# facebookresearch/jepa

Measured on NVIDIA H100. Metric: clips/sec ViT-L/16 16x224^2 synthetic V-JEPA pre-training step, higher is better.
Workload: dtype bf16

## Files before the change

### __graft_entry__.py

```python
import os
import sys

ROOT = os.path.dirname(os.path.abspath(__file__))
if ROOT not in sys.path:
    sys.path.insert(0, ROOT)


def build():
    from jepa_b200 import build as b
    b.build()
    import subprocess
    subprocess.check_call(["make", "-s", "-C", os.path.join(ROOT, "tests", "native"), "all", "test_xattn"])
    import jepa_b200
    from jepa_b200 import _lib
    _lib.load()
    import oracle.vjepa_oracle


def smoke():
    import torch
    sys.path.insert(0, os.path.join(ROOT, "tests"))
    sys.path.insert(0, os.path.join(ROOT, "tests", "golden"))
    from parity_util import run_c1_step_cuda, run_c1_step_oracle, compare_step
    assert torch.cuda.is_available(), "smoke() needs cuda:0"
    dev = torch.device("cuda:0")
    got = run_c1_step_cuda(dev, batch=1, depth_limit=2)
    ref = run_c1_step_oracle(batch=1, depth_limit=2)
    compare_step(got, ref, verbose=True)
    print("smoke OK: loss", got["loss_jepa"], "oracle", ref["loss_jepa"])


if __name__ == "__main__":
    build()
    if len(sys.argv) > 1 and sys.argv[1] == "smoke":
        smoke()
```

### jepa_b200/csrc/gemm.cu

```cuda

#include <stdlib.h>

#include "common.cuh"
#include "vjepa_b200.h"
#include "wgmma.cuh"

namespace vj {

constexpr int BM = 128;
constexpr int BK = 64;
constexpr int kGemmThreads = 384;
constexpr int kPromoteKB = 4;

struct GemmParams {
  int M, N, K;
  int tiles_m, tiles_n, split_k, kb_total, kb_per_split;
  int stream_k;
  long long sk_chunk;
  const float* bias;
  int epi;
  const void* aux;
  long long ldaux;
  const int* aux_rowmap;
  int aux_period;
  void* aux_out;
  long long ldauxout;
  void* D;
  long long ldd;
  int reduce_add;
  float alpha;
};

template <int BN>
struct GemmCfg {
  static constexpr int A_BYTES = BM * BK * 2;
  static constexpr int B_BYTES = BN * BK * 2;
  static constexpr int STAGE_BYTES = A_BYTES + B_BYTES;
  static constexpr int STAGES = BN == 256 ? 4 : (BN == 128 ? 6 : 8);
  static constexpr int BAR_OFF = STAGES * STAGE_BYTES;
  static constexpr int SMEM_BYTES = BAR_OFF + 2 * STAGES * 8 + 1024;
  static_assert(SMEM_BYTES <= 232448, "GEMM shared memory budget exceeded");
};

struct WorkCursor {
  long long cur, end;
};
VJ_DEVINL WorkCursor work_begin(const GemmParams& p) {
  WorkCursor c;
  if (p.stream_k) {
    const long long total_kb = (long long)p.tiles_m * p.tiles_n * p.kb_total;
    c.cur = (long long)blockIdx.x * p.sk_chunk;
    c.end = min(total_kb, c.cur + p.sk_chunk);
  } else {
    c.cur = blockIdx.x;
    c.end = (long long)p.tiles_m * p.tiles_n * p.split_k;
  }
  return c;
}
VJ_DEVINL bool work_next(const GemmParams& p, WorkCursor& c, int& t, int& kb0, int& kb1) {
  if (c.cur >= c.end) return false;
  if (p.stream_k) {
    t = int(c.cur / p.kb_total);
    kb0 = int(c.cur - (long long)t * p.kb_total);
    const long long take = min((long long)(p.kb_total - kb0), c.end - c.cur);
    kb1 = kb0 + int(take);
    c.cur += take;
  } else {
    const int tiles = p.tiles_m * p.tiles_n;
    const int split = int(c.cur / tiles);
    t = int(c.cur - (long long)split * tiles);
    kb0 = split * p.kb_per_split;
    kb1 = min(p.kb_total, kb0 + p.kb_per_split);
    c.cur += gridDim.x;
  }
  return true;
}

VJ_DEVINL float erf_as(float x) {
  const float ax = fabsf(x);
  const float t = __fdividef(1.0f, fmaf(0.3275911f, ax, 1.0f));
  float poly = fmaf(1.061405429f, t, -1.453152027f);
  poly = fmaf(poly, t, 1.421413741f);
  poly = fmaf(poly, t, -0.284496736f);
  poly = fmaf(poly, t, 0.254829592f);
  poly *= t;
  const float r = 1.0f - poly * __expf(-ax * ax);
  return copysignf(r, x);
}
VJ_DEVINL float gelu_and_grad(float x, float& d) {
  const float cdf = 0.5f * (1.0f + erf_as(x * 0.70710678118654752f));
  const float pdf = 0.39894228040143268f * __expf(-0.5f * x * x);
  d = fmaf(x, pdf, cdf);
  return x * cdf;
}
VJ_DEVINL float gelu_grad_fast(float x) {
  float d;
  gelu_and_grad(x, d);
  return d;
}

template <int BN, bool A_MN, bool B_MN, bool OUT_F32, int EPI, bool AUX32>
__global__ void __launch_bounds__(kGemmThreads, 1)
gemm_kernel(const __grid_constant__ CUtensorMap tmA, const __grid_constant__ CUtensorMap tmB, const GemmParams p) {
  constexpr bool kUsesAux = (EPI == VJ_EPI_ADD || EPI == VJ_EPI_DGELU || EPI == VJ_EPI_MUL);
  using Cfg = GemmCfg<BN>;
  constexpr int STAGES = Cfg::STAGES;
  extern __shared__ uint8_t smem_raw[];
  uint8_t* smem = reinterpret_cast<uint8_t*>((reinterpret_cast<uintptr_t>(smem_raw) + 1023) & ~uintptr_t(1023));
  uint64_t* bars = reinterpret_cast<uint64_t*>(smem + Cfg::BAR_OFF);
  const uint32_t full0 = smem_u32(bars);
  const uint32_t empty0 = smem_u32(bars + STAGES);
  const int wg = threadIdx.x >> 7;

  if (threadIdx.x == 0) {
    for (int s = 0; s < STAGES; ++s) {
      mbar_init(full0 + 8 * s, 1);
      mbar_init(empty0 + 8 * s, 8);
    }
    fence_mbar_init();
    tma_prefetch_desc(&tmA);
    tma_prefetch_desc(&tmB);
  }
  __syncthreads();

  if (wg == 0) {
    setmaxnreg_dec<40>();
    if (threadIdx.x == 0) {
      int stage = 0;
      uint32_t phase = 0;
      WorkCursor wc = work_begin(p);
      int t, kb0, kb1;
      while (work_next(p, wc, t, kb0, kb1)) {
        const int m0 = (t / p.tiles_n) * BM;
        const int n0 = (t % p.tiles_n) * BN;
        for (int kb = kb0; kb < kb1; ++kb) {
          mbar_wait(empty0 + 8 * stage, phase ^ 1);
          const uint32_t sa = smem_u32(smem + stage * Cfg::STAGE_BYTES);
          const uint32_t sb = sa + Cfg::A_BYTES;
          const uint32_t fb = full0 + 8 * stage;
          mbar_expect_tx(fb, Cfg::STAGE_BYTES);
          const int k0 = kb * BK;
          if (!A_MN) {
            tma_load_2d(sa, &tmA, fb, k0, m0);
          } else {
#pragma unroll
            for (int j = 0; j < BM / 64; ++j) tma_load_2d(sa + j * 8192, &tmA, fb, m0 + 64 * j, k0);
          }
          if (!B_MN) {
            tma_load_2d(sb, &tmB, fb, k0, n0);
          } else {
#pragma unroll
            for (int j = 0; j < BN / 64; ++j) tma_load_2d(sb + j * 8192, &tmB, fb, n0 + 64 * j, k0);
          }
          if (++stage == STAGES) {
            stage = 0;
            phase ^= 1;
          }
        }
      }
    }
    return;
  }

  setmaxnreg_inc<232>();
  const int cw = wg - 1;
  const int warp_in_wg = (threadIdx.x >> 5) & 3;
  const int lane = threadIdx.x & 31;
  constexpr bool kPromote = A_MN && B_MN;
  static_assert(!kPromote || BN <= 128, "promoted accumulation needs two accumulator sets in registers");
  int stage = 0;
  uint32_t phase = 0;
  float acc[BN / 2];
  float part[kPromote ? BN / 2 : 1];
  WorkCursor wc = work_begin(p);
  int t, kb0, kb1;
  while (work_next(p, wc, t, kb0, kb1)) {
    const int m0 = (t / p.tiles_n) * BM;
    const int n0 = (t % p.tiles_n) * BN;
    if constexpr (kPromote) {
#pragma unroll
      for (int i = 0; i < BN / 2; ++i) acc[i] = 0.f;
    }
    int prev = -1;
    for (int kb = kb0; kb < kb1; ++kb) {
      mbar_wait(full0 + 8 * stage, phase);
      const uint32_t sa = smem_u32(smem + stage * Cfg::STAGE_BYTES) + cw * 8192;
      const uint32_t sb = smem_u32(smem + stage * Cfg::STAGE_BYTES) + Cfg::A_BYTES;
      const uint64_t da0 = A_MN ? make_smem_desc(sa, 8192, 1024, 1) : make_smem_desc(sa, 16, 1024, 1);
      const uint64_t db0 = B_MN ? make_smem_desc(sb, 8192, 1024, 1) : make_smem_desc(sb, 16, 1024, 1);
      if constexpr (kPromote) {
        const bool group_first = (kb - kb0) % kPromoteKB == 0;
        const bool group_last = (kb - kb0) % kPromoteKB == kPromoteKB - 1 || kb + 1 == kb1;
        wgmma_fence_regs(part);
        wgmma_fence();
#pragma unroll
        for (int kk = 0; kk < BK / 16; ++kk)
          wgmma_ss<BN, 1, 1>(part, da0 + ((kk * 2048) >> 4), db0 + ((kk * 2048) >> 4), (!group_first || kk > 0) ? 1 : 0);
        wgmma_commit();
        if (group_last) {
          wgmma_wait<0>();
          wgmma_fence_regs(part);
#pragma unroll
          for (int i = 0; i < BN / 2; ++i) acc[i] += part[i];
        } else {
          wgmma_wait<1>();
        }
      } else {
        wgmma_fence_regs(acc);
        wgmma_fence();
#pragma unroll
        for (int kk = 0; kk < BK / 16; ++kk) {
          const uint32_t koa = A_MN ? kk * 2048 : kk * 32, kob = B_MN ? kk * 2048 : kk * 32;
          wgmma_ss<BN, A_MN ? 1 : 0, B_MN ? 1 : 0>(acc, da0 + (koa >> 4), db0 + (kob >> 4), (kb > kb0 || kk > 0) ? 1 : 0);
        }
        wgmma_commit();
        wgmma_wait<1>();
        wgmma_fence_regs(acc);
      }
      if (prev >= 0) {
        __syncwarp();
        if (lane == 0) mbar_arrive(empty0 + 8 * prev);
      }
      prev = stage;
      if (++stage == STAGES) {
        stage = 0;
        phase ^= 1;
      }
    }
    wgmma_wait<0>();
    wgmma_fence_regs(acc);
    __syncwarp();
    if (lane == 0) mbar_arrive(empty0 + 8 * prev);

    const bool add_bias = p.bias != nullptr && kb0 == 0;
    const int r0 = m0 + cw * 64 + warp_in_wg * 16 + (lane >> 2);
    const int cq = n0 + 2 * (lane & 3);
#pragma unroll
    for (int h = 0; h < 2; ++h) {
      const int row = r0 + 8 * h;
      if (row >= p.M) continue;
      long long arow = row;
      if (kUsesAux && AUX32) {
        if (p.aux_rowmap != nullptr) arow = p.aux_rowmap[row];
        else if (p.aux_period > 0) arow = row % p.aux_period;
      }
#pragma unroll
      for (int j = 0; j < BN / 8; ++j) {
        const int col = cq + 8 * j;
        float v0 = acc[4 * j + 2 * h] * p.alpha, v1 = acc[4 * j + 2 * h + 1] * p.alpha;
        if (add_bias) {
          const float2 b = __ldg(reinterpret_cast<const float2*>(p.bias + col));
          v0 += b.x;
          v1 += b.y;
        }
        if (kUsesAux) {
          float x0, x1;
          if (AUX32) {
            const float2 x = __ldg(reinterpret_cast<const float2*>(reinterpret_cast<const float*>(p.aux) + arow * p.ldaux + col));
            x0 = x.x; x1 = x.y;
          } else {
            const uint32_t x = __ldg(reinterpret_cast<const unsigned int*>(reinterpret_cast<const __nv_bfloat16*>(p.aux) +
                                                                             arow * p.ldaux + col));
            x0 = bf16_lo(x); x1 = bf16_hi(x);
          }
          if (EPI == VJ_EPI_ADD) { v0 += x0; v1 += x1; }
          else if (EPI == VJ_EPI_MUL) { v0 *= x0; v1 *= x1; }
          else { v0 *= gelu_grad_fast(x0); v1 *= gelu_grad_fast(x1); }
        }
        if (EPI == VJ_EPI_GELU || EPI == VJ_EPI_GELU_GRAD) {
          float d0, d1;
          const float g0 = gelu_and_grad(v0, d0), g1 = gelu_and_grad(v1, d1);
          if (p.aux_out != nullptr) {
            const uint32_t o = EPI == VJ_EPI_GELU ? pack_bf16x2(v0, v1) : pack_bf16x2(d0, d1);
            *reinterpret_cast<uint32_t*>(reinterpret_cast<__nv_bfloat16*>(p.aux_out) + (long long)row * p.ldauxout + col) = o;
          }
          v0 = g0;
          v1 = g1;
        }
        if (OUT_F32) {
          float2* dst = reinterpret_cast<float2*>(reinterpret_cast<float*>(p.D) + (long long)row * p.ldd + col);
          if (p.reduce_add) atomicAdd(dst, make_float2(v0, v1));
          else *dst = make_float2(v0, v1);
        } else {
          *reinterpret_cast<uint32_t*>(reinterpret_cast<__nv_bfloat16*>(p.D) + (long long)row * p.ldd + col) =
              pack_bf16x2(v0, v1);
        }
      }
    }
  }
}

template <int BN, bool A_MN, bool B_MN, bool OUT_F32, int EPI, bool AUX32 = false>
static int launch_gemm(const CUtensorMap& tA, const CUtensorMap& tB, const GemmParams& p, cudaStream_t stream) {
  using Cfg = GemmCfg<BN>;
  auto kern = gemm_kernel<BN, A_MN, B_MN, OUT_F32, EPI, AUX32>;
  static bool configured = false;
  if (!configured) {
    VJ_CUDA(cudaFuncSetAttribute(kern, cudaFuncAttributeMaxDynamicSharedMemorySize, Cfg::SMEM_BYTES));
    configured = true;
  }
  const int total = p.tiles_m * p.tiles_n * p.split_k;
  int grid = total < sm_budget() ? total : sm_budget();
  if (p.stream_k) {
    const long long total_kb = (long long)p.tiles_m * p.tiles_n * p.kb_total;
    grid = int((total_kb + p.sk_chunk - 1) / p.sk_chunk);
  }
  kern<<<grid, kGemmThreads, Cfg::SMEM_BYTES, stream>>>(tA, tB, p);
  VJ_CUDA(cudaGetLastError());
  vj::count_launch(1);
  return 0;
}

template <int BN>
static int dispatch_major(int a_mn, int b_mn, int out_f32, int epi, int aux_f32, const CUtensorMap& tA,
                          const CUtensorMap& tB, const GemmParams& p, cudaStream_t s) {
  if (!a_mn && !b_mn) {
    if (epi == VJ_EPI_NONE) return out_f32 ? launch_gemm<BN, false, false, true, VJ_EPI_NONE>(tA, tB, p, s)
                                           : launch_gemm<BN, false, false, false, VJ_EPI_NONE>(tA, tB, p, s);
    if (epi == VJ_EPI_ADD) {
      if (aux_f32) return out_f32 ? launch_gemm<BN, false, false, true, VJ_EPI_ADD, true>(tA, tB, p, s)
                                  : launch_gemm<BN, false, false, false, VJ_EPI_ADD, true>(tA, tB, p, s);
      if (!out_f32) return launch_gemm<BN, false, false, false, VJ_EPI_ADD, false>(tA, tB, p, s);
    }
    if (epi == VJ_EPI_GELU && !out_f32) return launch_gemm<BN, false, false, false, VJ_EPI_GELU>(tA, tB, p, s);
    if (epi == VJ_EPI_GELU_GRAD && !out_f32) return launch_gemm<BN, false, false, false, VJ_EPI_GELU_GRAD>(tA, tB, p, s);
    if (epi == VJ_EPI_DGELU && !out_f32 && !aux_f32) return launch_gemm<BN, false, false, false, VJ_EPI_DGELU>(tA, tB, p, s);
  } else if (!a_mn && b_mn) {
    if (epi == VJ_EPI_NONE) return out_f32 ? launch_gemm<BN, false, true, true, VJ_EPI_NONE>(tA, tB, p, s)
                                           : launch_gemm<BN, false, true, false, VJ_EPI_NONE>(tA, tB, p, s);
    if (epi == VJ_EPI_DGELU && !out_f32 && !aux_f32) return launch_gemm<BN, false, true, false, VJ_EPI_DGELU>(tA, tB, p, s);
    if (epi == VJ_EPI_MUL && !out_f32 && !aux_f32) return launch_gemm<BN, false, true, false, VJ_EPI_MUL>(tA, tB, p, s);
  } else if (a_mn && b_mn) {
    if constexpr (BN <= 128) {
      if (epi == VJ_EPI_NONE) return out_f32 ? launch_gemm<BN, true, true, true, VJ_EPI_NONE>(tA, tB, p, s)
                                             : launch_gemm<BN, true, true, false, VJ_EPI_NONE>(tA, tB, p, s);
    }
  }
  set_error("vj_gemm: combination a_mn=%d b_mn=%d d_f32=%d epi=%d is not instantiated", a_mn, b_mn, out_f32, epi);
  return -1;
}

}

extern "C" int vj_gemm(const void* A, long long lda, int a_mn, const void* B, long long ldb,
                       int b_mn, void* D, long long ldd, int d_f32, int M, int N, int K,
                       const float* bias, float alpha, int epi, const void* aux, long long ldaux,
                       int aux_f32, const int* aux_rowmap, int aux_period, void* aux_out,
                       long long ldauxout, int split_k, int accumulate, void* stream_) {
  using namespace vj;
  cudaStream_t stream = reinterpret_cast<cudaStream_t>(stream_);
  VJ_CHECK_ARG(A && B && D, "vj_gemm: null operand");
  VJ_CHECK_ARG(M > 0 && N > 0 && K > 0, "vj_gemm: empty problem M=%d N=%d K=%d", M, N, K);
  VJ_CHECK_ARG(N % 64 == 0, "vj_gemm: N=%d must be a multiple of 64", N);
  VJ_CHECK_ARG(lda % 8 == 0 && ldb % 8 == 0, "vj_gemm: lda/ldb must be multiples of 8 elements (16-byte rows)");
  VJ_CHECK_ARG(ldd % (d_f32 ? 4 : 8) == 0, "vj_gemm: ldd misaligned");
  VJ_CHECK_ARG((reinterpret_cast<uintptr_t>(A) & 15) == 0 && (reinterpret_cast<uintptr_t>(B) & 15) == 0 &&
                   (reinterpret_cast<uintptr_t>(D) & 15) == 0,
               "vj_gemm: operands must be 16-byte aligned");
  VJ_CHECK_ARG(epi >= VJ_EPI_NONE && epi <= VJ_EPI_GELU_GRAD, "vj_gemm: bad epilogue %d", epi);
  VJ_CHECK_ARG(!(accumulate || split_k > 1 || split_k < 0) || d_f32, "vj_gemm: accumulate/split-K needs fp32 D");
  VJ_CHECK_ARG(split_k >= 0 || (epi == VJ_EPI_NONE && accumulate), "vj_gemm: stream-K (split_k < 0) is for accumulating fp32 GEMMs");
  if (epi == VJ_EPI_ADD || epi == VJ_EPI_DGELU || epi == VJ_EPI_MUL) {
    VJ_CHECK_ARG(aux != nullptr, "vj_gemm: epilogue %d needs aux", epi);
    VJ_CHECK_ARG((reinterpret_cast<uintptr_t>(aux) & 15) == 0 && ldaux % (aux_f32 ? 4 : 8) == 0,
                 "vj_gemm: aux misaligned");
  }
  if (a_mn) VJ_CHECK_ARG(M % 8 == 0, "vj_gemm: MN-major A needs M %% 8 == 0");

  const int BN = (N % 256 == 0 && !(a_mn && b_mn)) ? 256 : (N % 128 == 0 ? 128 : 64);
  GemmParams p;
  p.M = M; p.N = N; p.K = K;
  p.tiles_m = (M + BM - 1) / BM;
  p.tiles_n = N / BN;
  p.kb_total = (K + BK - 1) / BK;
  p.stream_k = 0;
  p.sk_chunk = 0;
  if (split_k < 0) {
    const long long total_kb = (long long)p.tiles_m * p.tiles_n * p.kb_total;
    const long long ctas = total_kb < sm_budget() ? total_kb : sm_budget();
    p.stream_k = 1;
    p.sk_chunk = (total_kb + ctas - 1) / ctas;
    split_k = 1;
  }
  if (split_k < 1) split_k = 1;
  if (split_k > p.kb_total) split_k = p.kb_total;
  p.kb_per_split = (p.kb_total + split_k - 1) / split_k;
  p.split_k = (p.kb_total + p.kb_per_split - 1) / p.kb_per_split;
  p.bias = bias;
  p.epi = epi;
  p.aux = aux; p.ldaux = ldaux; p.aux_rowmap = aux_rowmap; p.aux_period = aux_period;
  p.aux_out = (epi == VJ_EPI_GELU || epi == VJ_EPI_GELU_GRAD) ? aux_out : nullptr;
  p.ldauxout = ldauxout;
  p.D = D; p.ldd = ldd;
  p.reduce_add = (accumulate || p.split_k > 1 || p.stream_k) ? 1 : 0;
  p.alpha = alpha;

  if (p.aux_out != nullptr)
    VJ_CHECK_ARG((reinterpret_cast<uintptr_t>(aux_out) & 3) == 0 && ldauxout % 2 == 0, "vj_gemm: aux_out misaligned");
  if ((epi == VJ_EPI_ADD || epi == VJ_EPI_DGELU || epi == VJ_EPI_MUL) && !aux_f32) {
    VJ_CHECK_ARG(aux_rowmap == nullptr && aux_period == 0, "vj_gemm: row-mapped / periodic aux must be fp32");
    VJ_CHECK_ARG(p.split_k == 1, "vj_gemm: aux epilogues do not combine with split-K");
  }
  CUtensorMap tA, tB;
  int rc;
  if (!a_mn) rc = make_tmap_2d(&tA, A, 0, K, M, lda * 2, 64, 128, 3);
  else       rc = make_tmap_2d(&tA, A, 0, M, K, lda * 2, 64, 64, 3);
  if (rc) return rc;
  if (!b_mn) rc = make_tmap_2d(&tB, B, 0, K, N, ldb * 2, 64, BN, 3);
  else       rc = make_tmap_2d(&tB, B, 0, N, K, ldb * 2, 64, 64, 3);
  if (rc) return rc;
  switch (BN) {
    case 256: return dispatch_major<256>(a_mn, b_mn, d_f32, epi, aux_f32, tA, tB, p, stream);
    case 128: return dispatch_major<128>(a_mn, b_mn, d_f32, epi, aux_f32, tA, tB, p, stream);
    default:  return dispatch_major<64>(a_mn, b_mn, d_f32, epi, aux_f32, tA, tB, p, stream);
  }
}
```

Before: 100.7.

## Add ping-pong consumer schedule and TMA-staged epilogue to GEMM kernel

Splits the GEMM kernel into a ping-pong variant, where two consumer warpgroups alternate tiles and hand off through named barriers, and a cooperative BN=256 variant used for long-K problems. The bf16 epilogue now stages results in swizzled shared memory and writes them with TMA stores. A producer thread prefetches bf16 aux tiles via TMA. The goal is to overlap one tile's epilogue with the next tile's MMA mainloop and to coalesce output writes. The cost is more shared memory for staging (fewer pipeline stages for some configs) and more complex synchronization. Weight-gradient (MN-major) GEMMs move to a separate kernel.

```diff
diff --git a/__graft_entry__.py b/__graft_entry__.py
--- a/__graft_entry__.py
+++ b/__graft_entry__.py
@@ -10,7 +10,8 @@
     from jepa_b200 import build as b
     b.build()
     import subprocess
-    subprocess.check_call(["make", "-s", "-C", os.path.join(ROOT, "tests", "native"), "all", "test_xattn"])
+    subprocess.check_call(["make", "-s", "-C", os.path.join(ROOT, "tests", "native"), "all", "test_xattn",
+                           "test_gemm_sched"])
     import jepa_b200
     from jepa_b200 import _lib
     _lib.load()
diff --git a/jepa_b200/csrc/gemm.cu b/jepa_b200/csrc/gemm.cu
--- a/jepa_b200/csrc/gemm.cu
+++ b/jepa_b200/csrc/gemm.cu
@@ -1,5 +1,6 @@
 
 #include <stdlib.h>
+#include <string.h>
 
 #include "common.cuh"
 #include "vjepa_b200.h"
@@ -10,6 +11,7 @@
 constexpr int BM = 128;
 constexpr int BK = 64;
 constexpr int kGemmThreads = 384;
+constexpr int kSmemBudget = 232448;
 constexpr int kPromoteKB = 4;
 
 struct GemmParams {
@@ -36,10 +38,28 @@
   static constexpr int A_BYTES = BM * BK * 2;
   static constexpr int B_BYTES = BN * BK * 2;
   static constexpr int STAGE_BYTES = A_BYTES + B_BYTES;
-  static constexpr int STAGES = BN == 256 ? 4 : (BN == 128 ? 6 : 8);
+  static constexpr int STAGES = BN == 128 ? 6 : 8;
   static constexpr int BAR_OFF = STAGES * STAGE_BYTES;
   static constexpr int SMEM_BYTES = BAR_OFF + 2 * STAGES * 8 + 1024;
-  static_assert(SMEM_BYTES <= 232448, "GEMM shared memory budget exceeded");
+  static_assert(SMEM_BYTES <= kSmemBudget, "GEMM shared memory budget exceeded");
+};
+
+template <int BN, bool STAGED, bool COOP>
+struct PingCfg {
+  static constexpr int ROWS = COOP ? 64 : BM;
+  static constexpr int A_BYTES = BM * BK * 2;
+  static constexpr int B_BYTES = BN * BK * 2;
+  static constexpr int STAGE_BYTES = A_BYTES + B_BYTES;
+  static constexpr int STG_BYTES = STAGED ? ROWS * BN * 2 : 0;
+  static constexpr int BAR_BYTES = 256;
+  static constexpr int FIT = (kSmemBudget - 1024 - BAR_BYTES - 2 * STG_BYTES) / STAGE_BYTES;
+  static constexpr int STAGES = FIT < 8 ? FIT : 8;
+  static constexpr int STG_OFF = STAGES * STAGE_BYTES;
+  static constexpr int BAR_OFF = STG_OFF + 2 * STG_BYTES;
+  static constexpr int SMEM_BYTES = BAR_OFF + BAR_BYTES + 1024;
+  static_assert(STAGES >= 3, "GEMM ring too shallow");
+  static_assert((2 * STAGES + 4) * 8 <= BAR_BYTES, "GEMM barrier block overflow");
+  static_assert(SMEM_BYTES <= kSmemBudget, "GEMM shared memory budget exceeded");
 };
 
 struct WorkCursor {
@@ -98,11 +118,305 @@
   gelu_and_grad(x, d);
   return d;
 }
-
-template <int BN, bool A_MN, bool B_MN, bool OUT_F32, int EPI, bool AUX32>
+template <int EPI>
+VJ_DEVINL void apply_aux(float& v0, float& v1, float x0, float x1) {
+  if (EPI == VJ_EPI_ADD) { v0 += x0; v1 += x1; }
+  else if (EPI == VJ_EPI_MUL) { v0 *= x0; v1 *= x1; }
+  else { v0 *= gelu_grad_fast(x0); v1 *= gelu_grad_fast(x1); }
+}
+VJ_DEVINL int aux32_row(const GemmParams& p, int row) {
+  if (row >= p.M) return 0;
+  if (p.aux_rowmap != nullptr) return p.aux_rowmap[row];
+  if (p.aux_period > 0) return row % p.aux_period;
+  return row;
+}
+
+template <int BN, bool OUT_F32, int EPI, bool AUX32>
+VJ_DEVINL void epilogue_direct(const GemmParams& p, const float (&acc)[BN / 2], int r0, int n0, bool add_bias, int lane) {
+  constexpr bool kUsesAux = (EPI == VJ_EPI_ADD || EPI == VJ_EPI_DGELU || EPI == VJ_EPI_MUL);
+  static_assert(!kUsesAux || AUX32, "bf16 aux goes through the staged epilogue");
+  const int cq = n0 + 2 * (lane & 3);
+#pragma unroll
+  for (int h = 0; h < 2; ++h) {
+    const int row = r0 + (lane >> 2) + 8 * h;
+    if (row >= p.M) continue;
+    const long long arow = kUsesAux ? aux32_row(p, row) : 0;
+#pragma unroll
+    for (int j = 0; j < BN / 8; ++j) {
+      const int col = cq + 8 * j;
+      float v0 = acc[4 * j + 2 * h] * p.alpha, v1 = acc[4 * j + 2 * h + 1] * p.alpha;
+      if (add_bias) {
+        const float2 b = __ldg(reinterpret_cast<const float2*>(p.bias + col));
+        v0 += b.x;
+        v1 += b.y;
+      }
+      if (kUsesAux) {
+        const float2 x = __ldg(reinterpret_cast<const float2*>(reinterpret_cast<const float*>(p.aux) + arow * p.ldaux + col));
+        apply_aux<EPI>(v0, v1, x.x, x.y);
+      }
+      if (OUT_F32) {
+        float2* dst = reinterpret_cast<float2*>(reinterpret_cast<float*>(p.D) + (long long)row * p.ldd + col);
+        if (p.reduce_add) atomicAdd(dst, make_float2(v0, v1));
+        else *dst = make_float2(v0, v1);
+      } else {
+        *reinterpret_cast<uint32_t*>(reinterpret_cast<__nv_bfloat16*>(p.D) + (long long)row * p.ldd + col) =
+            pack_bf16x2(v0, v1);
+      }
+    }
+  }
+}
+
+template <int BN, bool COOP, bool B_MN, bool OUT_F32, int EPI, bool AUX32>
 __global__ void __launch_bounds__(kGemmThreads, 1)
-gemm_kernel(const __grid_constant__ CUtensorMap tmA, const __grid_constant__ CUtensorMap tmB, const GemmParams p) {
+gemm_kernel(const __grid_constant__ CUtensorMap tmA, const __grid_constant__ CUtensorMap tmB,
+            const __grid_constant__ CUtensorMap tmD, const __grid_constant__ CUtensorMap tmAux,
+            const __grid_constant__ CUtensorMap tmAuxOut, const GemmParams p) {
   constexpr bool kUsesAux = (EPI == VJ_EPI_ADD || EPI == VJ_EPI_DGELU || EPI == VJ_EPI_MUL);
+  constexpr bool kStaged = !OUT_F32;
+  constexpr bool kAuxTma = kUsesAux && !AUX32;
+  constexpr bool kGelu = (EPI == VJ_EPI_GELU || EPI == VJ_EPI_GELU_GRAD);
+  static_assert(kStaged || !kAuxTma, "bf16 aux needs the staged epilogue");
+  static_assert(kStaged || !kGelu, "GELU epilogues write bf16");
+  using Cfg = PingCfg<BN, kStaged, COOP>;
+  constexpr int STAGES = Cfg::STAGES;
+  constexpr int ROWS = Cfg::ROWS;
+  constexpr int HALVES = ROWS / 64;
+  constexpr int kBlk = ROWS * 128;
+  extern __shared__ uint8_t smem_raw[];
+  uint8_t* smem = reinterpret_cast<uint8_t*>((reinterpret_cast<uintptr_t>(smem_raw) + 1023) & ~uintptr_t(1023));
+  uint64_t* bars = reinterpret_cast<uint64_t*>(smem + Cfg::BAR_OFF);
+  const uint32_t full0 = smem_u32(bars);
+  const uint32_t empty0 = smem_u32(bars + STAGES);
+  const uint32_t auxfull0 = smem_u32(bars + 2 * STAGES);
+  const uint32_t auxempty0 = smem_u32(bars + 2 * STAGES + 2);
+  const uint32_t stg0 = smem_u32(smem + Cfg::STG_OFF);
+  const int wg = threadIdx.x >> 7;
+
+  if (threadIdx.x == 0) {
+    for (int s = 0; s < STAGES; ++s) {
+      mbar_init(full0 + 8 * s, 1);
+      mbar_init(empty0 + 8 * s, COOP ? 8 : 4);
+    }
+    for (int c = 0; c < 2; ++c) {
+      mbar_init(auxfull0 + 8 * c, 1);
+      mbar_init(auxempty0 + 8 * c, 1);
+    }
+    fence_mbar_init();
+    tma_prefetch_desc(&tmA);
+    tma_prefetch_desc(&tmB);
+    if (kStaged) tma_prefetch_desc(&tmD);
+    if (kAuxTma) tma_prefetch_desc(&tmAux);
+  }
+  __syncthreads();
+
+  if (wg == 0) {
+    setmaxnreg_dec<40>();
+    WorkCursor wc = work_begin(p);
+    int t, kb0, kb1;
+    if (threadIdx.x == 0) {
+      int stage = 0;
+      uint32_t phase = 0;
+      while (work_next(p, wc, t, kb0, kb1)) {
+        const int m0 = (t / p.tiles_n) * BM;
+        const int n0 = (t % p.tiles_n) * BN;
+        for (int kb = kb0; kb < kb1; ++kb) {
+          mbar_wait(empty0 + 8 * stage, phase ^ 1);
+          const uint32_t sa = smem_u32(smem + stage * Cfg::STAGE_BYTES);
+          const uint32_t sb = sa + Cfg::A_BYTES;
+          const uint32_t fb = full0 + 8 * stage;
+          mbar_expect_tx(fb, Cfg::STAGE_BYTES);
+          const int k0 = kb * BK;
+          tma_load_2d(sa, &tmA, fb, k0, m0);
+          if (!B_MN) {
+            tma_load_2d(sb, &tmB, fb, k0, n0);
+          } else {
+#pragma unroll
+            for (int j = 0; j < BN / 64; ++j) tma_load_2d(sb + j * 8192, &tmB, fb, n0 + 64 * j, k0);
+          }
+          if (++stage == STAGES) {
+            stage = 0;
+            phase ^= 1;
+          }
+        }
+      }
+    } else if (kAuxTma && threadIdx.x == 32) {
+      for (int i = 0; work_next(p, wc, t, kb0, kb1); ++i) {
+        const int m0 = (t / p.tiles_n) * BM;
+        const int n0 = (t % p.tiles_n) * BN;
+#pragma unroll
+        for (int h = 0; h < (COOP ? 2 : 1); ++h) {
+          const int c = COOP ? h : (i & 1);
+          const uint32_t n = uint32_t(COOP ? i : (i >> 1));
+          mbar_wait(auxempty0 + 8 * c, (n & 1) ^ 1);
+          mbar_expect_tx(auxfull0 + 8 * c, Cfg::STG_BYTES);
+#pragma unroll
+          for (int j = 0; j < BN / 64; ++j)
+            tma_load_2d(stg0 + c * Cfg::STG_BYTES + j * kBlk, &tmAux, auxfull0 + 8 * c, n0 + 64 * j, m0 + ROWS * c * COOP);
+        }
+      }
+    }
+    return;
+  }
+
+  setmaxnreg_inc<232>();
+  const int cw = wg - 1;
+  const int warp_in_wg = (threadIdx.x >> 5) & 3;
+  const int lane = threadIdx.x & 31;
+  const bool elected = (threadIdx.x & 127) == 0;
+  const uint32_t stg = stg0 + cw * Cfg::STG_BYTES;
+  float acc[HALVES][BN / 2];
+  uint32_t ring_pos = 0;
+  uint32_t own = 0;
+  WorkCursor wc = work_begin(p);
+  int t, kb0, kb1;
+  for (int i = 0; work_next(p, wc, t, kb0, kb1); ++i) {
+    if (!COOP && (i & 1) != cw) {
+      ring_pos += kb1 - kb0;
+      continue;
+    }
+    WorkCursor peek = wc;
+    int t2, a2, b2;
+    const bool has_next = !COOP && work_next(p, peek, t2, a2, b2);
+    const int m0 = (t / p.tiles_n) * BM;
+    const int n0 = (t % p.tiles_n) * BN;
+    const int mw = m0 + (COOP ? 64 * cw : 0);
+
+    if (!COOP && i > 0) named_bar_sync(1 + cw, 256);
+    int stage = int(ring_pos % STAGES);
+    uint32_t phase = (ring_pos / STAGES) & 1;
+    int prev = -1;
+    for (int kb = kb0; kb < kb1; ++kb) {
+      mbar_wait(full0 + 8 * stage, phase);
+      const uint32_t sa = smem_u32(smem + stage * Cfg::STAGE_BYTES);
+      const uint32_t sb = sa + Cfg::A_BYTES;
+      const uint64_t da = make_smem_desc(sa + (COOP ? 8192 * cw : 0), 16, 1024, 1);
+      const uint64_t db = B_MN ? make_smem_desc(sb, 8192, 1024, 1) : make_smem_desc(sb, 16, 1024, 1);
+#pragma unroll
+      for (int hh = 0; hh < HALVES; ++hh) wgmma_fence_regs(acc[hh]);
+      wgmma_fence();
+#pragma unroll
+      for (int kk = 0; kk < BK / 16; ++kk) {
+        const uint32_t kob = B_MN ? kk * 2048 : kk * 32;
+        const int scale_d = (kb > kb0 || kk > 0) ? 1 : 0;
+#pragma unroll
+        for (int hh = 0; hh < HALVES; ++hh)
+          wgmma_ss<BN, 0, B_MN ? 1 : 0>(acc[hh], da + ((8192 * hh + kk * 32) >> 4), db + (kob >> 4), scale_d);
+      }
+      wgmma_commit();
+      wgmma_wait<1>();
+#pragma unroll
+      for (int hh = 0; hh < HALVES; ++hh) wgmma_fence_regs(acc[hh]);
+      if (prev >= 0) {
+        __syncwarp();
+        if (lane == 0) mbar_arrive(empty0 + 8 * prev);
+      }
+      prev = stage;
+      if (++stage == STAGES) {
+        stage = 0;
+        phase ^= 1;
+      }
+    }
+    ring_pos += kb1 - kb0;
+    if (has_next) named_bar_arrive(1 + (cw ^ 1), 256);
+    wgmma_wait<0>();
+#pragma unroll
+    for (int hh = 0; hh < HALVES; ++hh) wgmma_fence_regs(acc[hh]);
+    __syncwarp();
+    if (lane == 0) mbar_arrive(empty0 + 8 * prev);
+
+    const bool add_bias = p.bias != nullptr && kb0 == 0;
+    if constexpr (!kStaged) {
+#pragma unroll
+      for (int hh = 0; hh < HALVES; ++hh)
+        epilogue_direct<BN, OUT_F32, EPI, AUX32>(p, acc[hh], mw + 64 * hh + 16 * warp_in_wg, n0, add_bias, lane);
+    } else {
+      const int rq = lane >> 2;
+      const uint32_t thr = stg + (16 * warp_in_wg + rq) * 128 + 4 * (lane & 3);
+      if (kAuxTma) mbar_wait(auxfull0 + 8 * cw, own & 1);
+      else if (COOP) named_bar_sync(3 + cw, 128);
+      const bool two_pass = kGelu && p.aux_out != nullptr;
+#pragma unroll
+      for (int j = 0; j < BN / 8; ++j) {
+        const int col = n0 + 8 * j + 2 * (lane & 3);
+        float2 b = make_float2(0.f, 0.f);
+        if (add_bias) b = __ldg(reinterpret_cast<const float2*>(p.bias + col));
+        const uint32_t cj = thr + (j >> 3) * kBlk + (((j & 7) ^ rq) << 4);
+#pragma unroll
+        for (int hh = 0; hh < HALVES; ++hh)
+#pragma unroll
+          for (int h = 0; h < 2; ++h) {
+            const uint32_t addr = cj + (64 * hh + 8 * h) * 128;
+            float& a0 = acc[hh][4 * j + 2 * h];
+            float& a1 = acc[hh][4 * j + 2 * h + 1];
+            float v0 = a0 * p.alpha, v1 = a1 * p.alpha;
+            if (add_bias) {
+              v0 += b.x;
+              v1 += b.y;
+            }
+            if (kAuxTma) {
+              uint32_t x;
+              asm volatile("ld.shared.b32 %0, [%1];" : "=r"(x) : "r"(addr) : "memory");
+              apply_aux<EPI>(v0, v1, bf16_lo(x), bf16_hi(x));
+            } else if (kUsesAux) {
+              const long long arow = aux32_row(p, mw + 64 * hh + 16 * warp_in_wg + rq + 8 * h);
+              const float2 x = __ldg(reinterpret_cast<const float2*>(reinterpret_cast<const float*>(p.aux) +
+                                                                      arow * p.ldaux + col));
+              apply_aux<EPI>(v0, v1, x.x, x.y);
+            }
+            uint32_t o;
+            if (kGelu) {
+              float d0, d1;
+              const float g0 = gelu_and_grad(v0, d0), g1 = gelu_and_grad(v1, d1);
+              o = EPI == VJ_EPI_GELU ? pack_bf16x2(v0, v1) : pack_bf16x2(d0, d1);
+              a0 = g0;
+              a1 = g1;
+              if (!two_pass) o = pack_bf16x2(g0, g1);
+            } else {
+              o = pack_bf16x2(v0, v1);
+            }
+            asm volatile("st.shared.b32 [%0], %1;" ::"r"(addr), "r"(o) : "memory");
+          }
+      }
+      fence_proxy_async_smem();
+      named_bar_sync(3 + cw, 128);
+      if (two_pass) {
+        if (elected) {
+#pragma unroll
+          for (int j = 0; j < BN / 64; ++j) tma_store_2d(&tmAuxOut, stg + j * kBlk, n0 + 64 * j, mw);
+          tma_commit_group();
+          tma_wait_group_read<0>();
+        }
+        named_bar_sync(3 + cw, 128);
+#pragma unroll
+        for (int j = 0; j < BN / 8; ++j) {
+          const uint32_t cj = thr + (j >> 3) * kBlk + (((j & 7) ^ rq) << 4);
+#pragma unroll
+          for (int hh = 0; hh < HALVES; ++hh)
+#pragma unroll
+            for (int h = 0; h < 2; ++h) {
+              const uint32_t o = pack_bf16x2(acc[hh][4 * j + 2 * h], acc[hh][4 * j + 2 * h + 1]);
+              asm volatile("st.shared.b32 [%0], %1;" ::"r"(cj + (64 * hh + 8 * h) * 128), "r"(o) : "memory");
+            }
+        }
+        fence_proxy_async_smem();
+        named_bar_sync(3 + cw, 128);
+      }
+      if (elected) {
+#pragma unroll
+        for (int j = 0; j < BN / 64; ++j) tma_store_2d(&tmD, stg + j * kBlk, n0 + 64 * j, mw);
+        tma_commit_group();
+        tma_wait_group_read<0>();
+        if (kAuxTma) mbar_arrive(auxempty0 + 8 * cw);
+      }
+    }
+    ++own;
+  }
+}
+
+template <int BN, bool OUT_F32>
+__global__ void __launch_bounds__(kGemmThreads, 1)
+gemm_wgrad_kernel(const __grid_constant__ CUtensorMap tmA, const __grid_constant__ CUtensorMap tmB, const GemmParams p) {
+  static_assert(BN <= 128, "promoted accumulation needs two accumulator sets in registers");
   using Cfg = GemmCfg<BN>;
   constexpr int STAGES = Cfg::STAGES;
   extern __shared__ uint8_t smem_raw[];
@@ -140,18 +454,10 @@
           const uint32_t fb = full0 + 8 * stage;
           mbar_expect_tx(fb, Cfg::STAGE_BYTES);
           const int k0 = kb * BK;
-          if (!A_MN) {
-            tma_load_2d(sa, &tmA, fb, k0, m0);
-          } else {
-#pragma unroll
-            for (int j = 0; j < BM / 64; ++j) tma_load_2d(sa + j * 8192, &tmA, fb, m0 + 64 * j, k0);
-          }
-          if (!B_MN) {
-            tma_load_2d(sb, &tmB, fb, k0, n0);
-          } else {
-#pragma unroll
-            for (int j = 0; j < BN / 64; ++j) tma_load_2d(sb + j * 8192, &tmB, fb, n0 + 64 * j, k0);
-          }
+#pragma unroll
+          for (int j = 0; j < BM / 64; ++j) tma_load_2d(sa + j * 8192, &tmA, fb, m0 + 64 * j, k0);
+#pragma unroll
+          for (int j = 0; j < BN / 64; ++j) tma_load_2d(sb + j * 8192, &tmB, fb, n0 + 64 * j, k0);
           if (++stage == STAGES) {
             stage = 0;
             phase ^= 1;
@@ -166,56 +472,39 @@
   const int cw = wg - 1;
   const int warp_in_wg = (threadIdx.x >> 5) & 3;
   const int lane = threadIdx.x & 31;
-  constexpr bool kPromote = A_MN && B_MN;
-  static_assert(!kPromote || BN <= 128, "promoted accumulation needs two accumulator sets in registers");
   int stage = 0;
   uint32_t phase = 0;
   float acc[BN / 2];
-  float part[kPromote ? BN / 2 : 1];
+  float part[BN / 2];
   WorkCursor wc = work_begin(p);
   int t, kb0, kb1;
   while (work_next(p, wc, t, kb0, kb1)) {
     const int m0 = (t / p.tiles_n) * BM;
     const int n0 = (t % p.tiles_n) * BN;
-    if constexpr (kPromote) {
-#pragma unroll
-      for (int i = 0; i < BN / 2; ++i) acc[i] = 0.f;
-    }
+#pragma unroll
+    for (int i = 0; i < BN / 2; ++i) acc[i] = 0.f;
     int prev = -1;
     for (int kb = kb0; kb < kb1; ++kb) {
       mbar_wait(full0 + 8 * stage, phase);
       const uint32_t sa = smem_u32(smem + stage * Cfg::STAGE_BYTES) + cw * 8192;
       const uint32_t sb = smem_u32(smem + stage * Cfg::STAGE_BYTES) + Cfg::A_BYTES;
-      const uint64_t da0 = A_MN ? make_smem_desc(sa, 8192, 1024, 1) : make_smem_desc(sa, 16, 1024, 1);
-      const uint64_t db0 = B_MN ? make_smem_desc(sb, 8192, 1024, 1) : make_smem_desc(sb, 16, 1024, 1);
-      if constexpr (kPromote) {
-        const bool group_first = (kb - kb0) % kPromoteKB == 0;
-        const bool group_last = (kb - kb0) % kPromoteKB == kPromoteKB - 1 || kb + 1 == kb1;
+      const uint64_t da0 = make_smem_desc(sa, 8192, 1024, 1);
+      const uint64_t db0 = make_smem_desc(sb, 8192, 1024, 1);
+      const bool group_first = (kb - kb0) % kPromoteKB == 0;
+      const bool group_last = (kb - kb0) % kPromoteKB == kPromoteKB - 1 || kb + 1 == kb1;
+      wgmma_fence_regs(part);
+      wgmma_fence();
+#pragma unroll
+      for (int kk = 0; kk < BK / 16; ++kk)
+        wgmma_ss<BN, 1, 1>(part, da0 + ((kk * 2048) >> 4), db0 + ((kk * 2048) >> 4), (!group_first || kk > 0) ? 1 : 0);
+      wgmma_commit();
+      if (group_last) {
+        wgmma_wait<0>();
         wgmma_fence_regs(part);
-        wgmma_fence();
-#pragma unroll
-        for (int kk = 0; kk < BK / 16; ++kk)
-          wgmma_ss<BN, 1, 1>(part, da0 + ((kk * 2048) >> 4), db0 + ((kk * 2048) >> 4), (!group_first || kk > 0) ? 1 : 0);
-        wgmma_commit();
-        if (group_last) {
-          wgmma_wait<0>();
-          wgmma_fence_regs(part);
-#pragma unroll
-          for (int i = 0; i < BN / 2; ++i) acc[i] += part[i];
-        } else {
-          wgmma_wait<1>();
-        }
+#pragma unroll
+        for (int i = 0; i < BN / 2; ++i) acc[i] += part[i];
       } else {
-        wgmma_fence_regs(acc);
-        wgmma_fence();
-#pragma unroll
-        for (int kk = 0; kk < BK / 16; ++kk) {
-          const uint32_t koa = A_MN ? kk * 2048 : kk * 32, kob = B_MN ? kk * 2048 : kk * 32;
-          wgmma_ss<BN, A_MN ? 1 : 0, B_MN ? 1 : 0>(acc, da0 + (koa >> 4), db0 + (kob >> 4), (kb > kb0 || kk > 0) ? 1 : 0);
-        }
-        wgmma_commit();
         wgmma_wait<1>();
-        wgmma_fence_regs(acc);
       }
       if (prev >= 0) {
         __syncwarp();
@@ -233,107 +522,75 @@
     if (lane == 0) mbar_arrive(empty0 + 8 * prev);
 
     const bool add_bias = p.bias != nullptr && kb0 == 0;
-    const int r0 = m0 + cw * 64 + warp_in_wg * 16 + (lane >> 2);
-    const int cq = n0 + 2 * (lane & 3);
-#pragma unroll
-    for (int h = 0; h < 2; ++h) {
-      const int row = r0 + 8 * h;
-      if (row >= p.M) continue;
-      long long arow = row;
-      if (kUsesAux && AUX32) {
-        if (p.aux_rowmap != nullptr) arow = p.aux_rowmap[row];
-        else if (p.aux_period > 0) arow = row % p.aux_period;
-      }
-#pragma unroll
-      for (int j = 0; j < BN / 8; ++j) {
-        const int col = cq + 8 * j;
-        float v0 = acc[4 * j + 2 * h] * p.alpha, v1 = acc[4 * j + 2 * h + 1] * p.alpha;
-        if (add_bias) {
-          const float2 b = __ldg(reinterpret_cast<const float2*>(p.bias + col));
-          v0 += b.x;
-          v1 += b.y;
-        }
-        if (kUsesAux) {
-          float x0, x1;
-          if (AUX32) {
-            const float2 x = __ldg(reinterpret_cast<const float2*>(reinterpret_cast<const float*>(p.aux) + arow * p.ldaux + col));
-            x0 = x.x; x1 = x.y;
-          } else {
-            const uint32_t x = __ldg(reinterpret_cast<const unsigned int*>(reinterpret_cast<const __nv_bfloat16*>(p.aux) +
-                                                                             arow * p.ldaux + col));
-            x0 = bf16_lo(x); x1 = bf16_hi(x);
-          }
-          if (EPI == VJ_EPI_ADD) { v0 += x0; v1 += x1; }
-          else if (EPI == VJ_EPI_MUL) { v0 *= x0; v1 *= x1; }
-          else { v0 *= gelu_grad_fast(x0); v1 *= gelu_grad_fast(x1); }
-        }
-        if (EPI == VJ_EPI_GELU || EPI == VJ_EPI_GELU_GRAD) {
-          float d0, d1;
-          const float g0 = gelu_and_grad(v0, d0), g1 = gelu_and_grad(v1, d1);
-          if (p.aux_out != nullptr) {
-            const uint32_t o = EPI == VJ_EPI_GELU ? pack_bf16x2(v0, v1) : pack_bf16x2(d0, d1);
-            *reinterpret_cast<uint32_t*>(reinterpret_cast<__nv_bfloat16*>(p.aux_out) + (long long)row * p.ldauxout + col) = o;
-          }
-          v0 = g0;
-          v1 = g1;
-        }
-        if (OUT_F32) {
-          float2* dst = reinterpret_cast<float2*>(reinterpret_cast<float*>(p.D) + (long long)row * p.ldd + col);
-          if (p.reduce_add) atomicAdd(dst, make_float2(v0, v1));
-          else *dst = make_float2(v0, v1);
-        } else {
-          *reinterpret_cast<uint32_t*>(reinterpret_cast<__nv_bfloat16*>(p.D) + (long long)row * p.ldd + col) =
-              pack_bf16x2(v0, v1);
-        }
-      }
-    }
-  }
-}
-
-template <int BN, bool A_MN, bool B_MN, bool OUT_F32, int EPI, bool AUX32 = false>
-static int launch_gemm(const CUtensorMap& tA, const CUtensorMap& tB, const GemmParams& p, cudaStream_t stream) {
-  using Cfg = GemmCfg<BN>;
-  auto kern = gemm_kernel<BN, A_MN, B_MN, OUT_F32, EPI, AUX32>;
+    epilogue_direct<BN, OUT_F32, VJ_EPI_NONE, false>(p, acc, m0 + cw * 64 + warp_in_wg * 16, n0, add_bias, lane);
+  }
+}
+
+static int grid_size(const GemmParams& p) {
+  if (p.stream_k) {
+    const long long total_kb = (long long)p.tiles_m * p.tiles_n * p.kb_total;
+    return int((total_kb + p.sk_chunk - 1) / p.sk_chunk);
+  }
+  const int total = p.tiles_m * p.tiles_n * p.split_k;
+  return total < sm_budget() ? total : sm_budget();
+}
+
+struct GemmMaps {
+  CUtensorMap A, B, D, aux, aux_out;
+};
+
+template <int BN, bool COOP, bool B_MN, bool OUT_F32, int EPI, bool AUX32 = false>
+static int launch_gemm(const GemmMaps& m, const GemmParams& p, cudaStream_t stream) {
+  constexpr int SMEM = PingCfg<BN, !OUT_F32, COOP>::SMEM_BYTES;
+  auto kern = gemm_kernel<BN, COOP, B_MN, OUT_F32, EPI, AUX32>;
   static bool configured = false;
   if (!configured) {
-    VJ_CUDA(cudaFuncSetAttribute(kern, cudaFuncAttributeMaxDynamicSharedMemorySize, Cfg::SMEM_BYTES));
+    VJ_CUDA(cudaFuncSetAttribute(kern, cudaFuncAttributeMaxDynamicSharedMemorySize, SMEM));
     configured = true;
   }
-  const int total = p.tiles_m * p.tiles_n * p.split_k;
-  int grid = total < sm_budget() ? total : sm_budget();
-  if (p.stream_k) {
-    const long long total_kb = (long long)p.tiles_m * p.tiles_n * p.kb_total;
-    grid = int((total_kb + p.sk_chunk - 1) / p.sk_chunk);
-  }
-  kern<<<grid, kGemmThreads, Cfg::SMEM_BYTES, stream>>>(tA, tB, p);
+  kern<<<grid_size(p), kGemmThreads, SMEM, stream>>>(m.A, m.B, m.D, m.aux, m.aux_out, p);
   VJ_CUDA(cudaGetLastError());
   vj::count_launch(1);
   return 0;
 }
 
-template <int BN>
-static int dispatch_major(int a_mn, int b_mn, int out_f32, int epi, int aux_f32, const CUtensorMap& tA,
-                          const CUtensorMap& tB, const GemmParams& p, cudaStream_t s) {
+template <int BN, bool OUT_F32>
+static int launch_gemm_wgrad(const GemmMaps& m, const GemmParams& p, cudaStream_t stream) {
+  constexpr int SMEM = GemmCfg<BN>::SMEM_BYTES;
+  auto kern = gemm_wgrad_kernel<BN, OUT_F32>;
+  static bool configured = false;
+  if (!configured) {
+    VJ_CUDA(cudaFuncSetAttribute(kern, cudaFuncAttributeMaxDynamicSharedMemorySize, SMEM));
+    configured = true;
+  }
+  kern<<<grid_size(p), kGemmThreads, SMEM, stream>>>(m.A, m.B, p);
+  VJ_CUDA(cudaGetLastError());
+  vj::count_launch(1);
+  return 0;
+}
+
+template <int BN, bool COOP>
+static int dispatch_major(int a_mn, int b_mn, int out_f32, int epi, int aux_f32, const GemmMaps& m,
+                          const GemmParams& p, cudaStream_t s) {
   if (!a_mn && !b_mn) {
-    if (epi == VJ_EPI_NONE) return out_f32 ? launch_gemm<BN, false, false, true, VJ_EPI_NONE>(tA, tB, p, s)
-                                           : launch_gemm<BN, false, false, false, VJ_EPI_NONE>(tA, tB, p, s);
+    if (epi == VJ_EPI_NONE) return out_f32 ? launch_gemm<BN, COOP, false, true, VJ_EPI_NONE>(m, p, s)
+                                           : launch_gemm<BN, COOP, false, false, VJ_EPI_NONE>(m, p, s);
     if (epi == VJ_EPI_ADD) {
-      if (aux_f32) return out_f32 ? launch_gemm<BN, false, false, true, VJ_EPI_ADD, true>(tA, tB, p, s)
-                                  : launch_gemm<BN, false, false, false, VJ_EPI_ADD, true>(tA, tB, p, s);
-      if (!out_f32) return launch_gemm<BN, false, false, false, VJ_EPI_ADD, false>(tA, tB, p, s);
-    }
-    if (epi == VJ_EPI_GELU && !out_f32) return launch_gemm<BN, false, false, false, VJ_EPI_GELU>(tA, tB, p, s);
-    if (epi == VJ_EPI_GELU_GRAD && !out_f32) return launch_gemm<BN, false, false, false, VJ_EPI_GELU_GRAD>(tA, tB, p, s);
-    if (epi == VJ_EPI_DGELU && !out_f32 && !aux_f32) return launch_gemm<BN, false, false, false, VJ_EPI_DGELU>(tA, tB, p, s);
+      if (aux_f32) return out_f32 ? launch_gemm<BN, COOP, false, true, VJ_EPI_ADD, true>(m, p, s)
+                                  : launch_gemm<BN, COOP, false, false, VJ_EPI_ADD, true>(m, p, s);
+      if (!out_f32) return launch_gemm<BN, COOP, false, false, VJ_EPI_ADD, false>(m, p, s);
+    }
+    if (epi == VJ_EPI_GELU && !out_f32) return launch_gemm<BN, COOP, false, false, VJ_EPI_GELU>(m, p, s);
+    if (epi == VJ_EPI_GELU_GRAD && !out_f32) return launch_gemm<BN, COOP, false, false, VJ_EPI_GELU_GRAD>(m, p, s);
+    if (epi == VJ_EPI_DGELU && !out_f32 && !aux_f32) return launch_gemm<BN, COOP, false, false, VJ_EPI_DGELU>(m, p, s);
   } else if (!a_mn && b_mn) {
-    if (epi == VJ_EPI_NONE) return out_f32 ? launch_gemm<BN, false, true, true, VJ_EPI_NONE>(tA, tB, p, s)
-                                           : launch_gemm<BN, false, true, false, VJ_EPI_NONE>(tA, tB, p, s);
-    if (epi == VJ_EPI_DGELU && !out_f32 && !aux_f32) return launch_gemm<BN, false, true, false, VJ_EPI_DGELU>(tA, tB, p, s);
-    if (epi == VJ_EPI_MUL && !out_f32 && !aux_f32) return launch_gemm<BN, false, true, false, VJ_EPI_MUL>(tA, tB, p, s);
+    if (epi == VJ_EPI_NONE) return out_f32 ? launch_gemm<BN, COOP, true, true, VJ_EPI_NONE>(m, p, s)
+                                           : launch_gemm<BN, COOP, true, false, VJ_EPI_NONE>(m, p, s);
+    if (epi == VJ_EPI_DGELU && !out_f32 && !aux_f32) return launch_gemm<BN, COOP, true, false, VJ_EPI_DGELU>(m, p, s);
+    if (epi == VJ_EPI_MUL && !out_f32 && !aux_f32) return launch_gemm<BN, COOP, true, false, VJ_EPI_MUL>(m, p, s);
   } else if (a_mn && b_mn) {
-    if constexpr (BN <= 128) {
-      if (epi == VJ_EPI_NONE) return out_f32 ? launch_gemm<BN, true, true, true, VJ_EPI_NONE>(tA, tB, p, s)
-                                             : launch_gemm<BN, true, true, false, VJ_EPI_NONE>(tA, tB, p, s);
+    if constexpr (!COOP) {
+      if (epi == VJ_EPI_NONE) return out_f32 ? launch_gemm_wgrad<BN, true>(m, p, s) : launch_gemm_wgrad<BN, false>(m, p, s);
     }
   }
   set_error("vj_gemm: combination a_mn=%d b_mn=%d d_f32=%d epi=%d is not instantiated", a_mn, b_mn, out_f32, epi);
@@ -367,12 +624,15 @@
   }
   if (a_mn) VJ_CHECK_ARG(M % 8 == 0, "vj_gemm: MN-major A needs M %% 8 == 0");
 
-  const int BN = (N % 256 == 0 && !(a_mn && b_mn)) ? 256 : (N % 128 == 0 ? 128 : 64);
+  constexpr int kCoopMinKB = 48;
+  const int kb_total = (K + BK - 1) / BK;
+  const bool coop = !(a_mn && b_mn) && N % 256 == 0 && kb_total >= kCoopMinKB;
+  const int BN = coop ? 256 : (N % 128 == 0 ? 128 : 64);
   GemmParams p;
   p.M = M; p.N = N; p.K = K;
   p.tiles_m = (M + BM - 1) / BM;
   p.tiles_n = N / BN;
-  p.kb_total = (K + BK - 1) / BK;
+  p.kb_total = kb_total;
   p.stream_k = 0;
   p.sk_chunk = 0;
   if (split_k < 0) {
@@ -396,22 +656,28 @@
   p.alpha = alpha;
 
   if (p.aux_out != nullptr)
-    VJ_CHECK_ARG((reinterpret_cast<uintptr_t>(aux_out) & 3) == 0 && ldauxout % 2 == 0, "vj_gemm: aux_out misaligned");
-  if ((epi == VJ_EPI_ADD || epi == VJ_EPI_DGELU || epi == VJ_EPI_MUL) && !aux_f32) {
+    VJ_CHECK_ARG((reinterpret_cast<uintptr_t>(aux_out) & 15) == 0 && ldauxout % 8 == 0, "vj_gemm: aux_out misaligned");
+  const bool aux_tma = (epi == VJ_EPI_ADD || epi == VJ_EPI_DGELU || epi == VJ_EPI_MUL) && !aux_f32;
+  if (aux_tma) {
     VJ_CHECK_ARG(aux_rowmap == nullptr && aux_period == 0, "vj_gemm: row-mapped / periodic aux must be fp32");
     VJ_CHECK_ARG(p.split_k == 1, "vj_gemm: aux epilogues do not combine with split-K");
   }
-  CUtensorMap tA, tB;
+  GemmMaps m;
+  memset(&m, 0, sizeof(m));
   int rc;
-  if (!a_mn) rc = make_tmap_2d(&tA, A, 0, K, M, lda * 2, 64, 128, 3);
-  else       rc = make_tmap_2d(&tA, A, 0, M, K, lda * 2, 64, 64, 3);
+  if (!a_mn) rc = make_tmap_2d(&m.A, A, 0, K, M, lda * 2, 64, 128, 3);
+  else       rc = make_tmap_2d(&m.A, A, 0, M, K, lda * 2, 64, 64, 3);
   if (rc) return rc;
-  if (!b_mn) rc = make_tmap_2d(&tB, B, 0, K, N, ldb * 2, 64, BN, 3);
-  else       rc = make_tmap_2d(&tB, B, 0, N, K, ldb * 2, 64, 64, 3);
+  if (!b_mn) rc = make_tmap_2d(&m.B, B, 0, K, N, ldb * 2, 64, BN, 3);
+  else       rc = make_tmap_2d(&m.B, B, 0, N, K, ldb * 2, 64, 64, 3);
   if (rc) return rc;
-  switch (BN) {
-    case 256: return dispatch_major<256>(a_mn, b_mn, d_f32, epi, aux_f32, tA, tB, p, stream);
-    case 128: return dispatch_major<128>(a_mn, b_mn, d_f32, epi, aux_f32, tA, tB, p, stream);
-    default:  return dispatch_major<64>(a_mn, b_mn, d_f32, epi, aux_f32, tA, tB, p, stream);
-  }
-}
+  if (!(a_mn && b_mn) && !d_f32) {
+    const int rows = coop ? 64 : BM;
+    if ((rc = make_tmap_2d(&m.D, D, 0, N, M, ldd * 2, 64, rows, 3))) return rc;
+    if (aux_tma && (rc = make_tmap_2d(&m.aux, aux, 0, N, M, ldaux * 2, 64, rows, 3))) return rc;
+    if (p.aux_out != nullptr && (rc = make_tmap_2d(&m.aux_out, aux_out, 0, N, M, ldauxout * 2, 64, rows, 3))) return rc;
+  }
+  if (coop) return dispatch_major<256, true>(a_mn, b_mn, d_f32, epi, aux_f32, m, p, stream);
+  return BN == 128 ? dispatch_major<128, false>(a_mn, b_mn, d_f32, epi, aux_f32, m, p, stream)
+                   : dispatch_major<64, false>(a_mn, b_mn, d_f32, epi, aux_f32, m, p, stream);
+}
```

New measurement: 107.3, median of 6. 1.07x the previous value.
